# CommonRoad/commonroad-reactive-planner

Measured on AMD Instinct MI355X. Metric: candidate trajectories/sec (sample+cost+collision) per replan, higher is better.
Workload: dtype f64; 1 GPU; cfg3: DEU_Test-1_1_T-1, 31x31x63 grid, N=60, 51 obstacles (49 synthetic, seed 0); mode=draw, horizon_steps=60, n_obstacles=51, parallelism=one GPU, exchange=none

## Files before the change

### commonroad-reactive-planner_amd/csrc/rp_host.hip

```cpp
#include <hip/hip_runtime.h>
#include <hip/hip_ext.h>
#include <sched.h>

#include <algorithm>
#include <atomic>
#include <chrono>
#include <cmath>
#include <cstdio>
#include <cstdlib>
#include <cstring>
#include <mutex>
#include <new>
#include <string>
#include <unordered_map>
#include <vector>

#include "rp_kernels.h"
#include "rp_frontend.h"
#include "rp_corridor.h"
#include "rp_pool.h"

namespace {

constexpr int kBlocksPerCU = 4;
constexpr int kFoldPartials = 256;
constexpr int kFoldThreshold = 8192;
constexpr size_t kAutoMaterializeBytes = 64u << 20;
constexpr size_t kLdsTableLimit = 65536;
constexpr int kChunkMinWavesPerCU = 7;
constexpr int kCostMinPerCU = 832;
constexpr int kSweepMinPerCU = 512;
constexpr int kLazyCap[RP_LAZY_LEVELS] = {1024, 4096, 16384};
constexpr int kLazyOff[RP_LAZY_LEVELS] = {0, 1024, 5120};
constexpr int kLazyListWords = 21504;
constexpr uint32_t kLazyTarget[RP_LAZY_LEVELS] = {128, 1024, 8192};

using ResultBlock = FinalizeOut;

struct Options {
    int lanes = 0;
    int eval_block = 0;
    int cost_kernel = -1;
    int chunk_kernel = -1;
    int lazy = -1;
    int sweep = -1;
    int fused_lon = 1;
    int fused_lon_blocks = -1;
    int auto_materialize = 1;
    int stage_out = 1, row_padding = 1, row_align = 0, tail_split = 1;
    int table_window = 1;
    int fold_threshold = kFoldThreshold;
    int lon_publish = 1, inline_grids = 1, event_bracket = 0, winner_lanes_as_batch = 0, zero_copy = 1, coeff_groups = 1;
    int winner_skip_query = 1;
    int lazy_trace = 0, print_stamps = 0, timing = 0;
    int wait_mode = RP_WAIT_SPIN;
};
struct OptionDesc {
    const char *key;
    int Options::*field;
    const char *env;
    bool env_negates;
    int lo, hi;
};
const OptionDesc kOptionTable[] = {
    {"lanes", &Options::lanes, "RP_AMD_G", false, 0, 64},
    {"eval_block", &Options::eval_block, "RP_AMD_EVAL_BLOCK", false, 0, 256},
    {"cost_kernel", &Options::cost_kernel, "RP_AMD_COST_KERNEL", false, -1, 1},
    {"chunk_kernel", &Options::chunk_kernel, "RP_AMD_CHUNK_KERNEL", false, -1, 1},
    {"lazy", &Options::lazy, "RP_AMD_LAZY", false, -1, 1},
    {"sweep", &Options::sweep, "RP_AMD_SWEEP", false, -1, 1},
    {"fused_lon", &Options::fused_lon, "RP_AMD_NO_FUSED_LON", true, 0, 1},
    {"fused_lon_blocks", &Options::fused_lon_blocks, "RP_AMD_FUSED_LON_BLOCKS", false, -1, 1 << 20},
    {"auto_materialize", &Options::auto_materialize, "RP_AMD_NO_AUTO_MATERIALIZE", true, 0, 1},
    {"stage_out", &Options::stage_out, "RP_AMD_NO_STAGE_OUT", true, 0, 1},
    {"row_padding", &Options::row_padding, "RP_AMD_NO_ROW_PADDING", true, 0, 1},
    {"row_align", &Options::row_align, "RP_AMD_ROW_ALIGN", false, 0, 16},
    {"tail_split", &Options::tail_split, "RP_AMD_NO_TAIL_SPLIT", true, 0, 1},
    {"table_window", &Options::table_window, "RP_AMD_NO_TABLE_WINDOW", true, 0, 1},
    {"fold_threshold", &Options::fold_threshold, "RP_AMD_FOLD_THRESHOLD", false, 1, 1 << 30},
    {"lon_publish", &Options::lon_publish, "RP_AMD_NO_LON_PUBLISH", true, 0, 1},
    {"inline_grids", &Options::inline_grids, "RP_AMD_NO_INLINE_GRIDS", true, 0, 1},
    {"event_bracket", &Options::event_bracket, "RP_AMD_EVENT_BRACKET", false, 0, 1},
    {"winner_lanes_as_batch", &Options::winner_lanes_as_batch, "RP_AMD_WINNER_G_AS_BATCH", false, 0, 1},
    {"winner_skip_query", &Options::winner_skip_query, "RP_AMD_NO_WINNER_SKIP_QUERY", true, 0, 1},
    {"zero_copy", &Options::zero_copy, "RP_AMD_NO_ZERO_COPY", true, 0, 1},
    {"coeff_groups", &Options::coeff_groups, "RP_AMD_NO_COEFF_GROUPS", true, 0, 1},
    {"lazy_trace", &Options::lazy_trace, "RP_AMD_LAZY_TRACE", false, 0, 1},
    {"print_stamps", &Options::print_stamps, "RP_AMD_PRINT_STAMPS", false, 0, 1},
    {"timing", &Options::timing, "RP_AMD_TIMING", false, 0, 1},
    {"wait_mode", &Options::wait_mode, "RP_AMD_WAIT_MODE", false, RP_WAIT_SPIN, RP_WAIT_EVENT},
};
const OptionDesc *find_option(const char *key) {
    if (!key) return nullptr;
    for (const OptionDesc &d : kOptionTable)
        if (std::strcmp(d.key, key) == 0) return &d;
    return nullptr;
}
void options_from_environment(Options &o) {
    for (const OptionDesc &d : kOptionTable) {
        const char *e = d.env ? std::getenv(d.env) : nullptr;
        if (!e) continue;
        const int v = d.env_negates ? 0 : std::atoi(e);
        if (v >= d.lo && v <= d.hi) o.*(d.field) = v;
    }
}

}

struct rp_ctx {
    Options opt;
    int device = 0;
    hipStream_t stream = nullptr;
    std::string err;
    int num_cus = 256;
    int profiling = 0;
    unsigned long long calls = 0;
    hipEvent_t ev0 = nullptr, ev1 = nullptr;
    bool time_next_launch = false, timed_by_launch = false;

// ... 50 lines not shown
    std::chrono::steady_clock::time_point plan_t0;
    bool epilogue_dirty = false;
    struct Pending {
        bool active = false, cin = false, skip_eval = false, ticket = false, done = false, time_valid = false, mat = false, coeffs = false;
        unsigned long long seq = 0;
        int grid = 0;
        KArgs ka{};
        std::chrono::steady_clock::time_point tp0, tp1;
    } pending;
    struct LevelState {
        Pending pending;
        std::vector<char> staged;
        bool staged_on_device = false, last_rows_on_device = false;
        int last_G = 0, last_block = 0, last_kernel = 0, last_lazy = 0;
        size_t last_fused_lds = 0;
        int grid_index = 0;
    };
    std::vector<LevelState> chain;
    int chain_total = 0;
    unsigned long long *d_gate = nullptr;
    unsigned long long *d_sweep = nullptr;
    struct ChainInputs {
        rp_params p; rp_cost cost; std::vector<rp_grids> grids; std::vector<std::vector<double>> T, L, D; std::vector<std::vector<int32_t>> tl;
        int want = 0;
    } chain_in;
    int last_level = 0;
    char *d_result = nullptr, *h_result = nullptr, *h_result_dev = nullptr;
    size_t cap_result = 0;
    int64_t *d_single = nullptr, *h_single = nullptr;
    unsigned long long *d_debug = nullptr;
    unsigned long long seq = 0;
    bool spin_wait = true;
    hipEvent_t ev_done = nullptr;
    long long wait_fallbacks = 0;

    bool have_last = false, last_mat = false, last_coeffs = false;
    std::unordered_map<const void *, hipFunction_t> functions;
    std::vector<double> fast_buf;
    bool timing = false;
    double t_sum[6] = {0, 0, 0, 0, 0, 0};
    unsigned long long t_calls = 0;
    bool t_warm = false;
    std::chrono::steady_clock::time_point t_entry;
    bool last_rows_on_device = false;
    int last_G = 0;
    int last_block = 0;
    size_t last_fused_lds = 0;
    KArgs last{};
    KArgsG kargs_g{};
    KArgsGL kargs_gl{};
    bool grids_pending = false;
    char *h_arena = nullptr, *h_arena_dev = nullptr;
    int64_t arena_cap = 0;
    const double *cin_lon = nullptr, *cin_lat = nullptr;
    int64_t cin_groups = 0;
    const int32_t *cin_group_of = nullptr;
    int64_t cin_count = -1;
};

namespace {

int fail(rp_ctx *c, int code, const std::string &msg) {
    if (c) c->err = msg;
    return code;
}

// ... 75 lines not shown
        if (f && hipExtModuleLaunchKernel(f, (uint32_t)grid * (uint32_t)block, 1, 1, (uint32_t)block, 1, 1, lds, c->stream, nullptr, extra,
                                          c->ev0, c->ev1, 0) == hipSuccess) {
            c->timed_by_launch = true;
            return;
        }
        (void)hipGetLastError();
    }
    if (!f || hipModuleLaunchKernel(f, (unsigned)grid, 1, 1, (unsigned)block, 1, 1, (unsigned)lds, c->stream, nullptr, extra) != hipSuccess) {
        (void)hipGetLastError();
        void *args[] = {const_cast<void *>(args_block)};
        (void)hipLaunchKernel(kernel, dim3(grid), dim3(block), args, lds, c->stream);
    }
}

int collision_level(const KArgs &ka) {
    if (!ka.has_obstacles || (ka.flags & RP_FLAG_SKIP_COLLISION)) return 0;
    return (ka.obs.n_sobb + ka.obs.n_tri + ka.obs.n_circ) > 0 ? 2 : 1;
}

const void *sweep_kernel_fn(bool cin, int coll, bool one_chunk) {
    if (cin) {
        if (coll == 2) return one_chunk ? (const void *)rp_eval_kernel<16, false, true, 2, true, false, false, RP_BLOCK, true> : (const void *)rp_eval_kernel<16, false, true, 2, false, false, false, RP_BLOCK, true>;
        return one_chunk ? (const void *)rp_eval_kernel<16, false, true, 1, true, false, false, RP_BLOCK, true> : (const void *)rp_eval_kernel<16, false, true, 1, false, false, false, RP_BLOCK, true>;
    }
    if (coll == 2) return one_chunk ? (const void *)rp_eval_kernel<16, false, false, 2, true, false, false, RP_BLOCK, true> : (const void *)rp_eval_kernel<16, false, false, 2, false, false, false, RP_BLOCK, true>;
    return one_chunk ? (const void *)rp_eval_kernel<16, false, false, 1, true, false, false, RP_BLOCK, true> : (const void *)rp_eval_kernel<16, false, false, 1, false, false, false, RP_BLOCK, true>;
}

const void *chunk_kernel_fn(bool low, int coll) {
    if (low) return coll == 2 ? (const void *)rp_chunk_kernel<true, 2> : (coll == 1 ? (const void *)rp_chunk_kernel<true, 1> : (const void *)rp_chunk_kernel<true, 0>);
    return coll == 2 ? (const void *)rp_chunk_kernel<false, 2> : (coll == 1 ? (const void *)rp_chunk_kernel<false, 1> : (const void *)rp_chunk_kernel<false, 0>);
}

template <int G, bool MAT, bool CIN, int COLL, bool STAGE>
void launch_eval_tcs(rp_ctx *c, const KArgs &ka, int grid, size_t lds, int block = RP_BLOCK) {
    if constexpr (G == 16 && !STAGE) {
        if (block == 64) {
            if (ka.N + 1 <= G) launch_kargs(c, (const void *)rp_eval_kernel<G, MAT, CIN, COLL, true, false, false, 64>, grid, 64, lds, ka);
            else launch_kargs(c, (const void *)rp_eval_kernel<G, MAT, CIN, COLL, false, false, false, 64>, grid, 64, lds, ka);
            return;
        }
    }
    if (ka.N + 1 <= G) launch_kargs(c, (const void *)rp_eval_kernel<G, MAT, CIN, COLL, true, STAGE, false>, grid, RP_BLOCK, lds, ka);
    else launch_kargs(c, (const void *)rp_eval_kernel<G, MAT, CIN, COLL, false, STAGE, false>, grid, RP_BLOCK, lds, ka);
}

constexpr int kFusedLonG = 16;
constexpr size_t kFusedLonLdsLimit = 61440;
int fused_lon_max_blocks(const rp_ctx *c) {
    if (c->opt.fused_lon_blocks >= 0) return c->opt.fused_lon_blocks;
    return c->num_cus * 4;
}

size_t fused_lon_lds(const rp_ctx *c, const KArgs &ka, int64_t count, int G, bool cin, bool mat, int *pairs) {
    if (count <= 0 || !(G == kFusedLonG || (G == 64 && mat && ka.N + 1 <= 64) || (G == 32 && mat && ka.N + 1 <= 32))) return 0;
    const int gpb = RP_BLOCK / G;
    if ((count + gpb - 1) / gpb > (int64_t)fused_lon_max_blocks(c)) return 0;
    const int P = cin ? gpb : std::min<int64_t>(gpb, ((int64_t)gpb + ka.nD - 2) / ka.nD + 1);
    const size_t slot_bytes = ka.has_obstacles ? (size_t)ka.obs.n_clus * ka.obs.clus_per * RP_SLOT_ROW * sizeof(double) : 0;
    const size_t bytes = (size_t)ka.table_words * sizeof(double) + slot_bytes +
                         (size_t)P * ((size_t)PF_STRIDE * (size_t)(ka.N + 1) * sizeof(double) + sizeof(PairHdr) + sizeof(int) + sizeof(double)) + 16;
    if (bytes > kFusedLonLdsLimit) return 0;
    *pairs = P;
    return (bytes + 15) & ~(size_t)15;
}

template <bool MAT, bool CIN, int COLL>
void launch_eval_fused_c(rp_ctx *c, const KArgs &ka, int grid, size_t lds, int lanes) {
// ... 850 lines not shown
int rp_last_path(const rp_ctx *c) { return c ? c->last_lazy : 0; }
int rp_last_kernel(const rp_ctx *c) { return c ? c->last_kernel : 0; }

int rp_set_collision_path(rp_ctx *c, int mode) {
    if (!c) return RP_EINVAL;
    if (mode < RP_COLLISION_AUTO || mode > RP_COLLISION_TIMED) return fail(c, RP_EINVAL, "rp_set_collision_path: unknown mode");
    if (mode != c->collision_mode) { c->lazy_skip = c->lazy_penalty = 0; c->path_regime = -1; }
    c->collision_mode = mode;
    return RP_OK;
}

int rp_set_profiling(rp_ctx *c, int enable) {
    if (!c) return RP_EINVAL;
    c->profiling = enable < 0 ? 0 : enable;
    return RP_OK;
}

int rp_set_option(rp_ctx *c, const char *key, int64_t value) {
    if (!c) return RP_EINVAL;
    if (c->pending.active) return fail(c, RP_ESTATE, "rp_set_option: a plan is in flight on this context (rp_plan_wait first)");
    const OptionDesc *d = find_option(key);
    if (!d) return fail(c, RP_EINVAL, std::string("rp_set_option: unknown option '") + (key ? key : "(null)") + "'");
    if (value < d->lo || value > d->hi) return fail(c, RP_EINVAL, std::string("rp_set_option: value out of range for '") + key + "'");
    c->opt.*(d->field) = (int)value;
    c->timing = c->opt.timing != 0;
    c->spin_wait = c->opt.wait_mode != RP_WAIT_EVENT;
    c->lazy_skip = c->lazy_penalty = 0; c->path_regime = -1;
    return RP_OK;
}

int rp_get_option(const rp_ctx *c, const char *key, int64_t *value) {
    if (!c || !value) return RP_EINVAL;
    if (key && std::strcmp(key, "wait_fallbacks") == 0) { *value = c->wait_fallbacks; return RP_OK; }
    const OptionDesc *d = find_option(key);
    if (!d) return RP_EINVAL;
    *value = c->opt.*(d->field);
    return RP_OK;
}

int rp_set_wait_mode(rp_ctx *c, int mode) { return rp_set_option(c, "wait_mode", mode); }
int rp_get_wait_mode(const rp_ctx *c) { return c ? c->opt.wait_mode : RP_WAIT_SPIN; }

int rp_set_reference(rp_ctx *c, int32_t n, const double *ref_pos, const double *ref_theta, const double *ref_curv,
                     const double *ref_curv_d, const double *ref_x, const double *ref_y, double proj_domain_d_limit) {
    if (!c) return RP_EINVAL;
    if (c->pending.active) return fail(c, RP_ESTATE, "rp_set_reference: a plan is in flight on this context (rp_plan_wait first)");
    if (n < 2 || !ref_pos || !ref_theta || !ref_curv || !ref_curv_d || !ref_x || !ref_y)
        return fail(c, RP_EINVAL, "rp_set_reference: need n >= 2 and six non-null tables");
    for (int i = 0; i + 1 < n; ++i)
        if (!(ref_pos[i + 1] > ref_pos[i])) return fail(c, RP_EINVAL, "rp_set_reference: ref_pos must be strictly increasing");
    HIP_TRY(c, hipSetDevice(c->device));
    std::vector<double> t((size_t)TB_ROWS * (size_t)n);
    std::memcpy(&t[(size_t)TB_POS * n], ref_pos, sizeof(double) * n);
    std::memcpy(&t[(size_t)TB_THETA * n], ref_theta, sizeof(double) * n);
    std::memcpy(&t[(size_t)TB_CURV * n], ref_curv, sizeof(double) * n);
    std::memcpy(&t[(size_t)TB_CURV_D * n], ref_curv_d, sizeof(double) * n);
    std::memcpy(&t[(size_t)TB_X * n], ref_x, sizeof(double) * n);
    std::memcpy(&t[(size_t)TB_Y * n], ref_y, sizeof(double) * n);
    double *tx = &t[(size_t)TB_TX * n], *ty = &t[(size_t)TB_TY * n];
    std::vector<double> ux(n - 1), uy(n - 1);
    for (int i = 0; i + 1 < n; ++i) {
        double ex = ref_x[i + 1] - ref_x[i], ey = ref_y[i + 1] - ref_y[i];
        double ln = std::sqrt(ex * ex + ey * ey);
        if (!(ln > 0.0)) return fail(c, RP_EINVAL, "rp_set_reference: duplicate polyline vertices");
        ux[i] = ex / ln; uy[i] = ey / ln;
    }
// ... 1256 lines not shown
```

### commonroad-reactive-planner_amd/csrc/rp_kernels.h

```cpp
#pragma once

#include "rp_device.h"

#define RP_BLOCK 256
#ifndef RP_COPY_OUT_STORE
#define RP_COPY_OUT_STORE(p, v)                                                                                   \
    __builtin_nontemporal_store(*reinterpret_cast<const __attribute__((ext_vector_type(2))) double *>(&(v)),        \
                                reinterpret_cast<__attribute__((ext_vector_type(2))) double *>(p))
#endif
#ifndef RP_WRITE_THROUGH
#ifndef RP_BRANCHFREE_CONSTRAINTS
#define RP_BRANCHFREE_CONSTRAINTS 1
#endif
#define RP_WRITE_THROUGH 1
#endif
#ifndef RP_LATE_KERNARGS
#define RP_LATE_KERNARGS 1
#endif
#ifndef RP_WAVES_PER_SIMD
#define RP_WAVES_PER_SIMD 3
#endif

struct KArgs {
    double dt;
    int32_t N, factor, time_step0, low_vel_mode, lon_mode;
    uint32_t constraint_mask, flags;
    double x0_lon[3], x0_lat[3], x0_orientation;
    double wheelbase, wb_rear_axle, half_length, half_width, ego_radius;
    double a_max, v_switch, v_delta_max, kappa_max;
    double c_yaw;
    double c_kdot;
    int32_t cost_kind, has_speed, has_s, partials_cap;
    double w_a, desired_speed, desired_d, desired_s;
    int32_t nT, nL, nD, grids_inline;
    const double *T;
    const int32_t *traj_len;
    const double *L;
    const double *D;
    const double *lon_coeffs;
    const double *lat_coeffs;
    const int32_t *traj_len_c;
    const int32_t *pair_of;
    const int32_t *group_first;
    int64_t cand_begin, count;
    const int64_t *single_index;
    const int32_t *index_list;
    const uint32_t *list_count;
    int32_t list_cap;
    int32_t tail_split;
    struct LazyCtl *lazy_ctl;
    unsigned long long *sweep_init;
    unsigned long long *sweep_bound;
    int32_t partials_first, pad_sweep_;
// ... 1298 lines not shown
template <bool COEFFS_IN>
__device__ __forceinline__ void fetch_lateral(const KArgs &a, int64_t gidx, CandIn &ci, int64_t hdr_pair0) {
    int64_t pair;
    if (COEFFS_IN) {
        const double *pt = a.lat_coeffs + 6 * gidx;
#pragma unroll
        for (int k = 0; k < 6; ++k) ci.v[k] = pt[k];
        pair = pair_index<true>(a, gidx);
    } else {
        const uint32_t g32 = (uint32_t)gidx, nd = (uint32_t)a.nD;
        const uint32_t p32 = g32 / nd;
        pair = p32;
        ci.v[0] = grid_base(a)[a.nT + a.nL + (int)(g32 - p32 * nd)];
    }
    ci.pair_slot = pair - hdr_pair0;
}

__device__ __forceinline__ void fetch_header(const PairHdr *hdrs, CandIn &ci) {
    const PairHdr h = hdrs[ci.pair_slot];
    ci.lat_T = h.lat_T;
    ci.s0 = h.s0;
    ci.pre_reason = h.pre_reason;
    ci.L = h.L;
}

template <bool COEFFS_IN>
__device__ __forceinline__ CandIn fetch_candidate(const KArgs &a, int64_t gidx, const PairHdr *hdrs, int64_t hdr_pair0) {
    CandIn ci;
    fetch_lateral<COEFFS_IN>(a, gidx, ci, hdr_pair0);
    fetch_header(hdrs, ci);
    return ci;
}

template <int G, bool MAT, bool COEFFS_IN, int COLL, bool ONE_CHUNK, bool STAGE_OUT, bool LON_FUSED, int BLOCK = RP_BLOCK, bool SWEEP = false>
__global__ __launch_bounds__(BLOCK, RP_WAVES_PER_SIMD) void rp_eval_kernel(const KArgsG ag) {
    static_assert(!SWEEP || (G == 16 && !MAT && COLL != 0 && !STAGE_OUT && !LON_FUSED && BLOCK == RP_BLOCK), "the sweep's variant");
    const KArgs &a = ag.k;
    extern __shared__ double lds_out[];
    static_assert(!(LON_FUSED && STAGE_OUT), "the single-launch variant stores state rows directly");
    constexpr bool RP_WT = LON_FUSED && RP_WRITE_THROUGH;
    constexpr bool RP_NT = MAT && !LON_FUSED && !STAGE_OUT;
    touch_kernargs<10>();

    const int tid = threadIdx.x;
    RP_STAMP(0);
    RP_TL(0);
    const int lane = tid & 63;
    const int gl = lane & (G - 1);
    const int gbase = lane & ~(G - 1);
    static_assert(BLOCK == RP_BLOCK || (!LON_FUSED && !STAGE_OUT), "smaller workgroups: plain two-kernel variants only");
    constexpr int GPB = BLOCK / G;
    constexpr int GPW = 64 / G;
    constexpr int PFN = COLL ? PF_FIELDS : PF_COS_REF;
    const int wave_in_block = tid >> 6;
    const int group_in_wave = gbase / G;
    const int grp = tid / G;

    if (level_gate_closed(a.gate, a.gate_seq, a.gate_level)) return;
    if (a.single_index && *a.single_index < 0) {
        if (a.host_seq && a.ticket_if_none && tid == 0) __hip_atomic_store(a.host_seq, a.seq_value, __ATOMIC_RELEASE, __HIP_MEMORY_SCOPE_SYSTEM);
        return;
    }
    const int64_t wave_first = ((int64_t)blockIdx.x * GPB) + (int64_t)wave_in_block * GPW;
    int64_t count_ = a.single_index ? 1 : a.count;
    if (!LON_FUSED && a.index_list) {
        const uint32_t lc = *a.list_count;
        count_ = (int64_t)(lc < (uint32_t)a.list_cap ? lc : (uint32_t)a.list_cap);
        if ((int64_t)blockIdx.x * GPB >= count_) {
            if (a.partials) {
// ... 14 lines not shown
    if (sweep) {
        const int64_t sl = wave_first + group_in_wave;
        const bool v0 = sl < count;
        const int64_t slc = v0 ? sl : 0;
        const uint32_t st0 = a.status[slc];
        const double cs0 = a.cost[slc];
        const unsigned long long bound = __hip_atomic_load(a.sweep_bound, __ATOMIC_RELAXED, __HIP_MEMORY_SCOPE_AGENT);
        sweep_need = v0 && RP_STATUS_LABEL(st0) == RP_LABEL_FEASIBLE && cs0 == cs0 && cost_key(cs0) <= bound;
        __shared__ int sh_sweep_any;
        if (tid == 0) sh_sweep_any = 0;
        __syncthreads();
        if (__ballot(sweep_need) != 0 && lane == 0) sh_sweep_any = 1;
        __syncthreads();
        if (!sh_sweep_any) {
            if (a.partials) {
                const Partials bp = partials_at(a.partials, a.partials_cap, a.partials_first + (int)blockIdx.x);
                if (tid == 0) { bp.cost[0] = 0.0; bp.idx[0] = -1; }
                if (tid >= 8 && tid < 8 + RP_PARTIAL_CNT) bp.cnt[tid - 8] = 0u;
            }
            return;
        }
    }

    __shared__ GroupScratch sh_grp[GPB];
    __shared__ double sh_best_cost[GPB];
    __shared__ long long sh_best_idx[GPB];
    __shared__ int sh_cnt[10];

    const double *prof_base = a.profile;
    const PairHdr *hdr_base = a.pair_hdr;
    int64_t pair0 = a.pair_begin;
    CandIn cin;
    ProfStep pf0;
    const double *slot_lds = nullptr;
    if (LON_FUSED) {
        const int n0 = a.N + 1;
        double *const lds_tab = lds_out;
        double *const lds_prof = lds_tab + a.table_words;
        PairHdr *const lds_hdr = reinterpret_cast<PairHdr *>(lds_prof + (size_t)a.lds_pairs * PF_STRIDE * (size_t)n0);
        int *const lds_flags = reinterpret_cast<int *>(lds_hdr + a.lds_pairs);
        double *const lds_T = reinterpret_cast<double *>(lds_flags + ((a.lds_pairs + 1) & ~1));
        double *const lds_slot = reinterpret_cast<double *>((reinterpret_cast<uintptr_t>(lds_T + a.lds_pairs) + 15) & ~(uintptr_t)15);
        const int n_slots = (COLL == 2 && a.has_obstacles) ? a.obs.n_clus * a.obs.clus_per : 0;
        slot_lds = lds_slot;
        const int64_t s_first = (int64_t)blockIdx.x * GPB;
        const int64_t s_last = (s_first + GPB <= count ? s_first + GPB : count) - 1;
        const int64_t g_first = a.single_index ? *a.single_index : a.cand_begin + (s_first < count ? s_first : 0);
        const int64_t g_last = a.single_index ? g_first : a.cand_begin + (s_last >= s_first ? s_last : s_first);
        const int64_t p_first = COEFFS_IN ? g_first : (int64_t)((uint32_t)g_first / (uint32_t)a.nD);
        const int64_t p_last = COEFFS_IN ? g_last : (int64_t)((uint32_t)g_last / (uint32_t)a.nD);
        int P = (int)(p_last - p_first) + 1;
        P = P > a.lds_pairs ? a.lds_pairs : P;
        const int items = P * n0;
        __shared__ double sh_gT[GPB], sh_gL[GPB], sh_gD[GPB];
        __shared__ int sh_gtl[GPB];
        const int64_t slot0 = wave_first + group_in_wave;
        const int64_t g0 = a.single_index ? g_first : a.cand_begin + (slot0 < count ? slot0 : (wave_first < count ? wave_first : s_first));
        int j = lane;
        LonPairIn lin;
        double g_T = 0.0, g_L = 0.0, g_D = 0.0;
        int g_tl = 0;
        if (COEFFS_IN) {
            fetch_lateral<COEFFS_IN>(a, g0, cin, p_first);
            if (j < items) lin = lon_pair_fetch<COEFFS_IN>(a, p_first + (int)((uint32_t)j / (uint32_t)n0));
        } else {
            cin.pair_slot = (int64_t)((uint32_t)g0 / (uint32_t)a.nD) - p_first;
// ... 165 lines not shown
                RP_STAMP(22);
                const bool bounded = item_bound(it, bx, by, bR);
                RP_STAMP(23);
                if (!bounded) {
                    if (sub == 0 && dyn_here) atomicOr(mask_word(it, PF_NEAR), ~0ull);
                    continue;
                }
                if (dyn_here) {
                    uint64_t m = 0;
                    if (first) {
                        const double dx = f_cx - bx, dy = f_cy - by, rr = bR + f_r;
                        if (dx * dx + dy * dy <= rr * rr * 1.000001) m |= 1ull << (sub < 63 ? sub : 63);
                    }
                    for (int jo = sub + lanes_per_item; jo < ob.n_dyn; jo += lanes_per_item) {
                        const gcdouble o = dyn + (size_t)jo * ob.n_steps + kk;
                        const double dx = o[0] - bx, dy = o[plane] - by, rr = bR + o[6 * plane];
                        if (dx * dx + dy * dy <= rr * rr * 1.000001) m |= 1ull << (jo < 63 ? jo : 63);
                    }
                    if (m) atomicOr(mask_word(it, PF_NEAR), m);
                }
            }
            __syncthreads();
        }
        RP_STAMP(10);
        prof_base = lds_prof;
        hdr_base = lds_hdr;
        pair0 = p_first;
        pf0 = load_profile_item<PFN>(lds_prof + ((size_t)cin.pair_slot * (size_t)n0 + (size_t)(gl <= a.N ? gl : a.N)) * PF_STRIDE);
    } else {
        const int64_t slot0 = wave_first + group_in_wave;
        const int64_t ls0 = slot0 < count ? slot0 : (wave_first < count ? wave_first : (a.index_list ? (int64_t)blockIdx.x * GPB : 0));
        const int64_t g0 = a.single_index ? *a.single_index : (a.index_list ? (int64_t)a.index_list[ls0] : a.cand_begin + ls0);
        cin = fetch_candidate<COEFFS_IN>(a, g0, hdr_base, pair0);
        const int32_t ps0 = (int32_t)(pair_index<COEFFS_IN>(a, g0) - pair0);
        const int32_t pw0 = __builtin_amdgcn_readfirstlane(ps0);
        const uint32_t n80 = (uint32_t)(a.N + 1) * 8u;
        pf0 = load_profile<PFN, G == 16>(reinterpret_cast<const char *>(prof_base + ((size_t)pw0 * PF_FIELDS) * (size_t)(a.N + 1)),
                           (uint32_t)(ps0 - pw0) * PF_FIELDS * n80 + (uint32_t)(gl <= a.N ? gl : a.N) * 8u, n80);
    }

    if (!LON_FUSED) {
        if (tid < 10) sh_cnt[tid] = 0;
        if (tid < GPB) { sh_best_cost[tid] = 0.0; sh_best_idx[tid] = -1; }
        __syncthreads();
    }
    RP_STAMP(1);

    typedef const KArgs __attribute__((address_space(4))) *kargs_cptr;
    kargs_cptr ap_late = (LON_FUSED || MAT) ? (kargs_cptr)__builtin_amdgcn_kernarg_segment_ptr() : (kargs_cptr)&a;
    if (RP_LATE_KERNARGS && LON_FUSED) asm volatile("" : "+s"(ap_late));
    const KArgs __attribute__((address_space(4))) &al = *ap_late;
    const int N = al.N, n = N + 1;
    const int nchunks = ONE_CHUNK ? 1 : (n + G - 1) / G;
    const double dt = al.dt;
    const bool draw = (al.flags & RP_FLAG_DRAW_ALL) != 0;
    const bool low = al.low_vel_mode != 0;
    const uint32_t cm = al.constraint_mask;
    const int mid = n / 2;
    double *const gs_poly = sh_grp[grp].poly;
    double *const gs_last = sh_grp[grp].last;

    auto cost_terms = [&](int i, double acc, double v, double s, double d, double th_cl) -> double {
        double e, cst;
        e = al.w_a * acc; cst = e * e;
        e = 0.25 * (al.desired_d - d); cst = __builtin_fma(e, e, cst);
        e = 0.25 * fabs(th_cl); cst = __builtin_fma(e, e, cst);
        if (al.has_speed) { e = 5.0 * (v - al.desired_speed); cst = __builtin_fma(e, e, cst); }
        if (al.has_s) { e = 0.25 * (al.desired_s - s); cst = __builtin_fma(e, e, cst); }
        if (i == N) {
            e = 20.0 * (al.desired_d - d); cst = __builtin_fma(e, e, cst);
            e = 5.0 * fabs(th_cl); cst = __builtin_fma(e, e, cst);
            if (al.has_speed) { e = v - al.desired_speed; cst += 50.0 * (e * e); }
            if (al.has_s) { e = 20.0 * (al.desired_s - s); cst = __builtin_fma(e, e, cst); }
        }
        if (i == mid && al.has_speed) { e = v - al.desired_speed; cst += 100.0 * (e * e); }
        return cst;
    };

    if (wave_first < count) {
        const int64_t w0 = wave_first;
        const int64_t slot = w0 + group_in_wave;
        const bool valid = slot < count && sweep_need;
        const int64_t gidx = al.single_index ? *al.single_index
                             : ((!LON_FUSED && al.index_list) ? (int64_t)al.index_list[valid ? slot : w0] : al.cand_begin + (valid ? slot : w0));

        const int L = cin.L;
        const double s0 = cin.s0;
        const uint32_t pre_reason = (uint32_t)cin.pre_reason;
        const int32_t pair_slot_ = (int32_t)(pair_index<COEFFS_IN>(al, gidx) - pair0);
        const int32_t pair_w = __builtin_amdgcn_readfirstlane(pair_slot_);
        const uint32_t n8p = (uint32_t)n * 8u;
        const char *const pbase = reinterpret_cast<const char *>(prof_base + ((size_t)pair_w * PF_FIELDS) * (size_t)n);
        const uint32_t poff8 = (uint32_t)(pair_slot_ - pair_w) * PF_FIELDS * n8p;
        ProfStep pf = pf0;
        if (!LON_FUSED) {
            Poly lat;
            if (COEFFS_IN) lat = {cin.v[0], cin.v[1], cin.v[2], cin.v[3], cin.v[4], cin.v[5]};
            else lat = quintic_coeffs(al.x0_lat[0], al.x0_lat[1], al.x0_lat[2], cin.v[0], 0.0, 0.0, cin.lat_T);
            if (gl == 0) park_poly(gs_poly, lat);
        }
        RP_STAMP(2);

        int fail_step = -1, ood_step = -1;
        uint32_t fail_reason = RP_REASON_NONE;
        bool collide = false;
        double cost_acc = 0.0;

        bool alive = valid && pre_reason == RP_REASON_NONE;
        if (__ballot(alive) != 0) {
            double theta_carry = al.x0_orientation;
            double kappa_carry = 0.0;
            double cumx = 0.0, cumy = 0.0;
            const bool store_ok = MAT && valid && pre_reason == RP_REASON_NONE;
            const int ns = (MAT && !STAGE_OUT) ? al.row_stride : n;
            constexpr bool SPLIT_OK = MAT && !STAGE_OUT && !LON_FUSED && G == 16;
            const int tail_m = SPLIT_OK ? al.tail_split : 0;
            const uint32_t cand8 = (uint32_t)state_block_doubles(ns, tail_m) * 8u;
            char *const obase = !MAT ? nullptr
                                : (STAGE_OUT ? reinterpret_cast<char *>(lds_out + (size_t)(wave_in_block * GPW) * RP_N_ARRAYS * (size_t)n)
                                             : reinterpret_cast<char *>(al.states) + (size_t)w0 * (size_t)cand8);
            const uint32_t n8 = (uint32_t)ns * 8u;
            const uint32_t lane_off8 = (uint32_t)group_in_wave * (STAGE_OUT ? RP_N_ARRAYS * n8 : cand8);
            constexpr bool ROW_MULV = LON_FUSED;
            constexpr bool LATE_STORE = MAT && !STAGE_OUT;
            uint32_t n8v = n8;
            auto row_at = [&](uint32_t off8, int row) -> double * {
                return reinterpret_cast<double *>(obase + (size_t)(ROW_MULV ? __umul24((uint32_t)row, n8v) + off8 : off8 + (uint32_t)row * n8));
            };

#pragma nounroll
            for (int c = 0; c < nchunks; ++c) {
                const int base = c * G;
                const int i = base + gl;
                const bool live = i <= N;
                const bool act = i < L;
                if (ROW_MULV) asm volatile("" : "+v"(n8v));

                if (!ONE_CHUNK && c > 0) {
                    if (LON_FUSED) pf = load_profile_item<PFN>(prof_base + ((size_t)pair_slot_ * (size_t)n + (size_t)(live ? i : N)) * PF_STRIDE);
                    else pf = load_profile<PFN, G == 16>(pbase, poff8 + (uint32_t)(live ? i : N) * 8u, n8p);
                }
                double s = pf.f[PF_S], sd = pf.f[PF_SD], sdd = pf.f[PF_SDD];
                const double inv_sd = pf.f[PF_INV_SD], th_ref = pf.f[PF_TH_REF];
                const double k_r = pf.f[PF_KR], k_r_d = pf.f[PF_KRD];
                const double px = pf.f[PF_PX], py = pf.f[PF_PY], nx = pf.f[PF_NX], ny = pf.f[PF_NY];
                const bool s_in_dom = pf.f[PF_INDOM] != 0.0;

                constexpr bool SKIP_EXTENDED = !(MAT && COLL == 0);
                double d = 0.0, dd = 0.0, ddd = 0.0, th_cl = 0.0, th_gl = 0.0, cos_gl = 1.0, sin_gl = 0.0;
                double kappa = 0.0, v = 0.0, acc = 0.0, kdot = 0.0, x = 0.0, y = 0.0;
                uint64_t near_sta_cell = 0;
                if (!SKIP_EXTENDED || __any(act)) {
                    const double t = (double)i * dt;
                    const double tau = low ? s - s0 : t;
                    d = poly_pos(gs_poly, tau); dd = poly_vel(gs_poly, tau); ddd = poly_acc(gs_poly, tau);
                    if (fabs(dd) < RP_EPS) dd = 0.0;
                    if (!LATE_STORE && store_ok && act) {
                        const uint32_t off8 = lane_off8 + (uint32_t)i * 8u;
                        st_row<RP_WT, RP_NT>(row_at(off8, RP_S), s);
                        st_row<RP_WT, RP_NT>(row_at(off8, RP_S_DOT), sd);
                        st_row<RP_WT, RP_NT>(row_at(off8, RP_S_DDOT), sdd);
                        st_row<RP_WT, RP_NT>(row_at(off8, RP_D), d);
                        st_row<RP_WT, RP_NT>(row_at(off8, RP_D_DOT), dd);
                        st_row<RP_WT, RP_NT>(row_at(off8, RP_D_DDOT), ddd);
                    }
                    RP_STAMP(3);

                    const bool moving = inv_sd > 0.0;
                    double dp, dpp;
                    if (!low) {
                        dp = dd * inv_sd;
                        const double ddot = ddd - dp * sdd;
                        dpp = ddot * inv_sd * inv_sd;
                    } else {
                        dp = dd;
                        dpp = ddd;
                    }

                    const bool use_atan = moving || low;
                    th_cl = rp_atan(dp);
                    th_gl = th_cl + th_ref;
                    const double w2 = __builtin_fma(dp, dp, 1.0);
                    double cosT = rp_rsqrt(w2);
                    double secT = w2 * cosT;
                    double tanT = dp;
                    if (__any(act && !use_atan)) {
                        const uint64_t mv = group_ballot<G>(use_atan && act, gbase);
                        const uint64_t below = mv & ((1ull << gl) - 1ull);
                        const int src = below ? 63 - __clzll(below) : 0;
                        const double th_from = group_bcast<G>(th_gl, src);
                        if (!use_atan) {
                            th_gl = below ? th_from : theta_carry;
                            th_cl = th_gl - th_ref;
                        }
                        double sn, cs;
                        rp_sincos(th_cl, &sn, &cs);
                        const double sc = rp_rcp(cs);
                        cosT = use_atan ? cosT : cs;
                        secT = use_atan ? secT : sc;
                        tanT = use_atan ? tanT : sn * sc;
                    }
                    const double sinT = tanT * cosT;
                    cos_gl = heading_cos(pf.f[PF_COS_REF], pf.f[PF_SIN_REF], cosT, sinT);
                    sin_gl = heading_sin(pf.f[PF_COS_REF], pf.f[PF_SIN_REF], cosT, sinT);
                    RP_STAMP(5);

                    const double oneKrD = 1.0 - k_r * d;
                    const double q = cosT * rp_rcp(oneKrD);
                    const double kterm = frenet_kterm(k_r_d, d, k_r, dp);
                    kappa = frenet_kappa(dpp, kterm, tanT, cosT, q, k_r);
                    const double f = oneKrD * secT;
                    v = sd * f;
                    acc = frenet_acc(sdd, f, sd, secT, oneKrD, tanT, kappa, k_r, kterm);

                    double th_prev = lane_prev(th_gl), ka_prev = lane_prev(kappa);
                    if (gl == 0) { th_prev = theta_carry; ka_prev = kappa_carry; }
                    const double dth = i > 0 ? th_gl - th_prev : 0.0;
                    kdot = i > 0 ? kappa - ka_prev : 0.0;
                    RP_STAMP(6);

    #if RP_BRANCHFREE_CONSTRAINTS
                    uint32_t reason = RP_REASON_NONE;
                    {
                        const double a_max = al.a_max, v_switch = al.v_switch, kappa_max = al.kappa_max;
                        const double wk = al.wheelbase * kappa;
                        const bool bad_yaw = fabs(rint(dth * al.c_yaw)) > kappa_max * v * 1e5;
                        const bool bad_kd = fabs(kdot) > al.c_kdot * __builtin_fma(wk, wk, 1.0);
                        const bool fast = v > v_switch;
                        const double acc_l = fast ? acc * v : acc, acc_r = fast ? a_max * v_switch : a_max;
                        const bool bad_acc = !((-a_max <= acc) & (acc_l <= acc_r));
                        const bool bad_v = v < -RP_EPS, bad_k = fabs(kappa) > kappa_max;
                        reason = (((cm & RP_CHECK_ACCELERATION) != 0) & bad_acc) ? RP_REASON_ACCELERATION : reason;
                        reason = (((cm & RP_CHECK_KAPPA_DOT) != 0) & bad_kd) ? RP_REASON_KAPPA_DOT : reason;
                        reason = (((cm & RP_CHECK_YAW_RATE) != 0) & bad_yaw) ? RP_REASON_YAW_RATE : reason;
                        reason = (((cm & RP_CHECK_KAPPA) != 0) & bad_k) ? RP_REASON_KAPPA : reason;
                        reason = (((cm & RP_CHECK_VELOCITY) != 0) & bad_v) ? RP_REASON_VELOCITY : reason;
                        reason = act ? reason : RP_REASON_NONE;
                    }
    #else
                    uint32_t reason = RP_REASON_NONE;
                    if (act) {
                        const double wk = al.wheelbase * kappa;
                        const bool bad_yaw = fabs(rint(dth * al.c_yaw)) > al.kappa_max * v * 1e5;
                        const bool bad_kd = fabs(kdot) > al.c_kdot * __builtin_fma(wk, wk, 1.0);
                        const bool ok_acc = (-al.a_max <= acc) && (v > al.v_switch ? acc * v <= al.a_max * al.v_switch : acc <= al.a_max);
                        if ((cm & RP_CHECK_VELOCITY) && v < -RP_EPS) reason = RP_REASON_VELOCITY;
                        else if ((cm & RP_CHECK_KAPPA) && fabs(kappa) > al.kappa_max) reason = RP_REASON_KAPPA;
                        else if ((cm & RP_CHECK_YAW_RATE) && bad_yaw) reason = RP_REASON_YAW_RATE;
                        else if ((cm & RP_CHECK_KAPPA_DOT) && bad_kd) reason = RP_REASON_KAPPA_DOT;
                        else if ((cm & RP_CHECK_ACCELERATION) && !ok_acc) reason = RP_REASON_ACCELERATION;
                    }
    #endif
                    if (__any(reason != RP_REASON_NONE)) {
                        const uint64_t fm = group_ballot<G>(reason != RP_REASON_NONE, gbase);
                        const int fl = fm ? __ffsll((unsigned long long)fm) - 1 : 0;
                        const uint32_t r_first = (uint32_t)__shfl((int)reason, fl, G);
                        if (fm && fail_step < 0) { fail_step = base + fl; fail_reason = r_first; }
                        if (!draw && fail_step >= 0) alive = false;
                        if (__ballot(alive) == 0) break;
                    }
                    RP_STAMP(7);

                    const bool in_dom = s_in_dom && fabs(d) <= al.proj_d_limit;
                    x = px + d * nx; y = py + d * ny;
                    if (__any(act && !in_dom) || ood_step >= 0) {
                        const uint64_t om = group_ballot<G>(act && !in_dom, gbase);
                        if (om && ood_step < 0) ood_step = base + __ffsll((unsigned long long)om) - 1;
                        if (ood_step >= 0 && i >= ood_step) { x = 0.0; y = 0.0; }
                    }
                    if (act) {
                        if (!LATE_STORE && store_ok) {
                            const uint32_t off8 = lane_off8 + (uint32_t)i * 8u;
                            st_row<RP_WT, RP_NT>(row_at(off8, RP_X), x);
                            st_row<RP_WT, RP_NT>(row_at(off8, RP_Y), y);
                            st_row<RP_WT, RP_NT>(row_at(off8, RP_THETA), th_gl);
                            st_row<RP_WT, RP_NT>(row_at(off8, RP_V), v);
                            st_row<RP_WT, RP_NT>(row_at(off8, RP_A), acc);
                            st_row<RP_WT, RP_NT>(row_at(off8, RP_KAPPA), kappa);
                            st_row<RP_WT, RP_NT>(row_at(off8, RP_KAPPA_DOT), kdot);
                            st_row<RP_WT, RP_NT>(row_at(off8, RP_THETA_CL), th_cl);
                        }
                        cost_acc += cost_terms(i, acc, v, s, d, th_cl);
                    }
                    if (COLL == 2 && live && alive && fail_step < 0 && ood_step < 0 && !collide && act)
                        near_sta_cell = static_grid_mask(al.obs.grid, al.obs.gx0, al.obs.gy0, al.obs.ginv, al.obs.gnx, al.obs.gny,
                                                         x + al.wb_rear_axle * cos_gl, y + al.wb_rear_axle * sin_gl);
                }
                const bool cell_wanted = COLL == 2 && live && alive && fail_step < 0 && ood_step < 0 && !collide;
                RP_STAMP(8);

                const int ll = L - 1 - base;
                const bool take = (ll >= 0 && ll < G);
                if (__any(take && L < n)) {
                    if (!COLL) rp_sincos(th_gl, &sin_gl, &cos_gl);
                    if (take && gl == ll) {
                        double *o = gs_last;
                        o[0] = x; o[1] = y; o[2] = th_gl; o[3] = v; o[4] = acc; o[5] = kappa; o[6] = kdot;
// ... 71 lines not shown
                        char *const tbase = obase + (size_t)(lane_off8 + (uint32_t)(RP_N_ARRAYS * tail_m) * 8u + (uint32_t)gl * 8u);
                        const bool lo = gl < 8;
                        auto pair_store = [&](int q, double r0, double r1) {
                            const double up = dpp_f64<DPP_ROW_SHR8, 0xf>(r1);
                            st_row<RP_WT, RP_NT>(reinterpret_cast<double *>(tbase + q * 128), lo ? r0 : up);
                        };
                        pair_store(0, x, y); pair_store(1, th_gl, v); pair_store(2, acc, kappa); pair_store(3, kdot, s);
                        pair_store(4, d, th_cl); pair_store(5, sd, sdd); pair_store(6, dd, ddd);
                    }
                } else
                if (LATE_STORE && store_ok && i < ns) {
                    const uint32_t off8 = lane_off8 + (uint32_t)i * 8u;
                    st_row<RP_WT, RP_NT>(row_at(off8, RP_X), x);
                    st_row<RP_WT, RP_NT>(row_at(off8, RP_Y), y);
                    st_row<RP_WT, RP_NT>(row_at(off8, RP_THETA), th_gl);
                    st_row<RP_WT, RP_NT>(row_at(off8, RP_V), v);
                    st_row<RP_WT, RP_NT>(row_at(off8, RP_A), acc);
                    st_row<RP_WT, RP_NT>(row_at(off8, RP_KAPPA), kappa);
                    st_row<RP_WT, RP_NT>(row_at(off8, RP_KAPPA_DOT), kdot);
                    st_row<RP_WT, RP_NT>(row_at(off8, RP_S), s);
                    st_row<RP_WT, RP_NT>(row_at(off8, RP_D), d);
                    st_row<RP_WT, RP_NT>(row_at(off8, RP_THETA_CL), th_cl);
                    st_row<RP_WT, RP_NT>(row_at(off8, RP_S_DOT), sd);
                    st_row<RP_WT, RP_NT>(row_at(off8, RP_S_DDOT), sdd);
                    st_row<RP_WT, RP_NT>(row_at(off8, RP_D_DOT), dd);
                    st_row<RP_WT, RP_NT>(row_at(off8, RP_D_DDOT), ddd);
                }
                RP_STAMP(9);

                if (COLL) {
                    const bool want = live && alive && fail_step < 0 && ood_step < 0 && !collide;
                    bool hit = false;
                    constexpr bool masked = !COEFFS_IN;
                    const uint64_t near_dyn = double_as_mask(pf.f[PF_NEAR]);
                    const double ego_cx = x + al.wb_rear_axle * cos_gl, ego_cy = y + al.wb_rear_axle * sin_gl;
                    const uint64_t near_sta = want ? near_sta_cell : 0;
                    const bool ask = want && ((!masked && al.obs.n_dyn > 0) || (near_dyn | near_sta) != 0);
                    RP_STAMP(44);
#ifdef RP_WALK_COUNT
                    if (a.debug && !a.single_index && blockIdx.x == RP_STAMP_BLOCK && threadIdx.x == RP_STAMP_THREAD) rp_walk_dbg = a.debug + 40;
#endif
                    if (__any(ask)) {
                        ObsTables ob;
                        ob.sobb = al.obs.sobb; ob.tri = al.obs.tri; ob.circ = al.obs.circ; ob.dyn = al.obs.dyn;
                        ob.clus = al.obs.clus; ob.clus_info = al.obs.clus_info;
                        ob.n_sobb = al.obs.n_sobb; ob.n_tri = al.obs.n_tri; ob.n_circ = al.obs.n_circ; ob.n_dyn = al.obs.n_dyn;
                        ob.n_steps = al.obs.n_steps; ob.dyn_t0 = al.obs.dyn_t0; ob.n_clus = al.obs.n_clus; ob.clus_per = al.obs.clus_per;
                        ob.dyn_rmax_all = al.obs.dyn_rmax_all;
                        const Obb ego = {ego_cx, ego_cy, cos_gl, sin_gl, al.half_length, al.half_width};
                        RP_STAMP(45);
                        hit = pose_collides<masked, COLL == 2, LON_FUSED && COLL == 2, true, !MAT>(ob, ego, al.ego_radius, al.time_step0 + i * al.factor, ask,
                                                                                             near_dyn, near_sta, slot_lds) && ask;
                    }
                    RP_STAMP(46);
                    collide |= group_ballot<G>(hit, gbase) != 0;
                }
                RP_STAMP(11);
            }
        }
        RP_STAMP(12);
        if (MAT && STAGE_OUT) {
            const uint64_t okmask = __ballot(valid && pre_reason == RP_REASON_NONE);
            if (okmask) {
                const int blk2 = (RP_N_ARRAYS * n) >> 1;
                const double2 *src = reinterpret_cast<const double2 *>(lds_out + (size_t)(wave_in_block * GPW) * RP_N_ARRAYS * (size_t)n);
                double2 *dst = reinterpret_cast<double2 *>(al.states + ((size_t)w0 * RP_N_ARRAYS) * (size_t)n);
                for (int k = lane; k < GPW * blk2; k += 64) {
// ... 842 lines not shown
```

Measured before the change: 455.5 million candidates/s.

## Stage per-pair reference profile rows in LDS for the two-kernel eval path

Adds a PROF_LDS kernel variant that cooperatively copies each workgroup's longitudinal profile rows from global memory into LDS once, in batched loads, transposed to a strided per-step layout. The per-step loop then reads profile fields from LDS as needed, instead of reloading them from global memory for every chunk. This is meant to cut repeated global profile traffic and register pressure in the materialized, non-coefficient path. In exchange it adds LDS allocation (capped at 32KB), which may lower occupancy, plus a prologue copy. An option can disable it.

Result: faster. 464.3 million candidates/s (median of 6 runs) (+1.9%).

```diff
diff --git a/commonroad-reactive-planner_amd/csrc/rp_host.hip b/commonroad-reactive-planner_amd/csrc/rp_host.hip
--- a/commonroad-reactive-planner_amd/csrc/rp_host.hip
+++ b/commonroad-reactive-planner_amd/csrc/rp_host.hip
@@ -52,6 +52,7 @@
     int fold_threshold = kFoldThreshold;
     int lon_publish = 1, inline_grids = 1, event_bracket = 0, winner_lanes_as_batch = 0, zero_copy = 1, coeff_groups = 1;
     int winner_skip_query = 1;
+    int profile_lds = 1;
     int lazy_trace = 0, print_stamps = 0, timing = 0;
     int wait_mode = RP_WAIT_SPIN;
 };
@@ -85,6 +86,7 @@
     {"winner_skip_query", &Options::winner_skip_query, "RP_AMD_NO_WINNER_SKIP_QUERY", true, 0, 1},
     {"zero_copy", &Options::zero_copy, "RP_AMD_NO_ZERO_COPY", true, 0, 1},
     {"coeff_groups", &Options::coeff_groups, "RP_AMD_NO_COEFF_GROUPS", true, 0, 1},
+    {"profile_lds", &Options::profile_lds, "RP_AMD_NO_PROFILE_LDS", true, 0, 1},
     {"lazy_trace", &Options::lazy_trace, "RP_AMD_LAZY_TRACE", false, 0, 1},
     {"print_stamps", &Options::print_stamps, "RP_AMD_PRINT_STAMPS", false, 0, 1},
     {"timing", &Options::timing, "RP_AMD_TIMING", false, 0, 1},
@@ -201,6 +203,7 @@
     unsigned long long seq = 0;
     bool spin_wait = true;
     hipEvent_t ev_done = nullptr;
+    long long prof_lds_launches = 0;
     long long wait_fallbacks = 0;
 
     bool have_last = false, last_mat = false, last_coeffs = false;
@@ -342,8 +345,30 @@
     return coll == 2 ? (const void *)rp_chunk_kernel<false, 2> : (coll == 1 ? (const void *)rp_chunk_kernel<false, 1> : (const void *)rp_chunk_kernel<false, 0>);
 }
 
+constexpr size_t kProfLdsLimit = 32768;
+size_t prof_lds_bytes(const rp_ctx *c, const KArgs &ka, int G, int block, int *pairs) {
+    if (!c->opt.profile_lds || G != 16 || block != RP_BLOCK || ka.N + 1 <= G || ka.single_index || ka.index_list || ka.nD <= 0) return 0;
+    const int gpb = RP_BLOCK / G;
+    const int P = (int)std::min<int64_t>(gpb, ((int64_t)gpb + ka.nD - 2) / ka.nD + 1);
+    const size_t bytes = (size_t)P * PF_STRIDE * (size_t)(ka.N + 1) * sizeof(double);
+    if (bytes > kProfLdsLimit) return 0;
+    *pairs = P;
+    return bytes;
+}
+
 template <int G, bool MAT, bool CIN, int COLL, bool STAGE>
 void launch_eval_tcs(rp_ctx *c, const KArgs &ka, int grid, size_t lds, int block = RP_BLOCK) {
+    if constexpr (G == 16 && MAT && !CIN && !STAGE) {
+        int pairs = 0;
+        const size_t bytes = prof_lds_bytes(c, ka, G, block, &pairs);
+        if (bytes) {
+            KArgs kp = ka;
+            kp.lds_pairs = pairs;
+            launch_kargs(c, (const void *)rp_eval_kernel<G, MAT, CIN, COLL, false, false, false, RP_BLOCK, false, true>, grid, RP_BLOCK, bytes, kp);
+            ++c->prof_lds_launches;
+            return;
+        }
+    }
     if constexpr (G == 16 && !STAGE) {
         if (block == 64) {
             if (ka.N + 1 <= G) launch_kargs(c, (const void *)rp_eval_kernel<G, MAT, CIN, COLL, true, false, false, 64>, grid, 64, lds, ka);
@@ -1260,6 +1285,7 @@
 int rp_get_option(const rp_ctx *c, const char *key, int64_t *value) {
     if (!c || !value) return RP_EINVAL;
     if (key && std::strcmp(key, "wait_fallbacks") == 0) { *value = c->wait_fallbacks; return RP_OK; }
+    if (key && std::strcmp(key, "profile_lds_launches") == 0) { *value = c->prof_lds_launches; return RP_OK; }
     const OptionDesc *d = find_option(key);
     if (!d) return RP_EINVAL;
     *value = c->opt.*(d->field);
diff --git a/commonroad-reactive-planner_amd/csrc/rp_kernels.h b/commonroad-reactive-planner_amd/csrc/rp_kernels.h
--- a/commonroad-reactive-planner_amd/csrc/rp_kernels.h
+++ b/commonroad-reactive-planner_amd/csrc/rp_kernels.h
@@ -19,6 +19,9 @@
 #endif
 #ifndef RP_WAVES_PER_SIMD
 #define RP_WAVES_PER_SIMD 3
+#endif
+#ifndef RP_PROF_LDS_WAVES
+#define RP_PROF_LDS_WAVES 3
 #endif
 
 struct KArgs {
@@ -1383,9 +1386,12 @@
     return ci;
 }
 
-template <int G, bool MAT, bool COEFFS_IN, int COLL, bool ONE_CHUNK, bool STAGE_OUT, bool LON_FUSED, int BLOCK = RP_BLOCK, bool SWEEP = false>
-__global__ __launch_bounds__(BLOCK, RP_WAVES_PER_SIMD) void rp_eval_kernel(const KArgsG ag) {
+template <int G, bool MAT, bool COEFFS_IN, int COLL, bool ONE_CHUNK, bool STAGE_OUT, bool LON_FUSED, int BLOCK = RP_BLOCK, bool SWEEP = false,
+          bool PROF_LDS = false>
+__global__ __launch_bounds__(BLOCK, PROF_LDS ? RP_PROF_LDS_WAVES : RP_WAVES_PER_SIMD) void rp_eval_kernel(const KArgsG ag) {
     static_assert(!SWEEP || (G == 16 && !MAT && COLL != 0 && !STAGE_OUT && !LON_FUSED && BLOCK == RP_BLOCK), "the sweep's variant");
+    static_assert(!PROF_LDS || (G == 16 && !COEFFS_IN && !ONE_CHUNK && !STAGE_OUT && !LON_FUSED && BLOCK == RP_BLOCK && !SWEEP),
+                  "profile rows in LDS: 16-lane grid plans of the two-kernel path, 256-thread workgroups");
     const KArgs &a = ag.k;
     extern __shared__ double lds_out[];
     static_assert(!(LON_FUSED && STAGE_OUT), "the single-launch variant stores state rows directly");
@@ -1466,6 +1472,7 @@
     int64_t pair0 = a.pair_begin;
     CandIn cin;
     ProfStep pf0;
+    int32_t plds0 = 0;
     const double *slot_lds = nullptr;
     if (LON_FUSED) {
         const int n0 = a.N + 1;
@@ -1697,11 +1704,37 @@
         const int64_t ls0 = slot0 < count ? slot0 : (wave_first < count ? wave_first : (a.index_list ? (int64_t)blockIdx.x * GPB : 0));
         const int64_t g0 = a.single_index ? *a.single_index : (a.index_list ? (int64_t)a.index_list[ls0] : a.cand_begin + ls0);
         cin = fetch_candidate<COEFFS_IN>(a, g0, hdr_base, pair0);
-        const int32_t ps0 = (int32_t)(pair_index<COEFFS_IN>(a, g0) - pair0);
-        const int32_t pw0 = __builtin_amdgcn_readfirstlane(ps0);
-        const uint32_t n80 = (uint32_t)(a.N + 1) * 8u;
-        pf0 = load_profile<PFN, G == 16>(reinterpret_cast<const char *>(prof_base + ((size_t)pw0 * PF_FIELDS) * (size_t)(a.N + 1)),
-                           (uint32_t)(ps0 - pw0) * PF_FIELDS * n80 + (uint32_t)(gl <= a.N ? gl : a.N) * 8u, n80);
+        if (PROF_LDS) {
+            const int n0 = a.N + 1;
+            const int64_t s_first = (int64_t)blockIdx.x * GPB, s_last = (s_first + GPB <= count ? s_first + GPB : count) - 1;
+            const uint32_t nd = (uint32_t)a.nD, p_first = (uint32_t)(a.cand_begin + s_first) / nd;
+            const int P = (int)((uint32_t)(a.cand_begin + s_last) / nd - p_first) + 1;
+            plds0 = (int32_t)((int64_t)p_first - pair0);
+            const int rows = (P < a.lds_pairs ? P : a.lds_pairs) * PFN;
+            const double *const src = prof_base + (size_t)plds0 * PF_FIELDS * (size_t)n0;
+            constexpr int WPB = BLOCK / 64, BATCH = 8;
+            for (int r0 = wave_in_block; r0 < rows; r0 += BATCH * WPB) {
+                for (int i = lane; i < n0; i += 64) {
+                    double v[BATCH];
+#pragma unroll
+                    for (int u = 0; u < BATCH; ++u) {
+                        const int r = r0 + u * WPB < rows ? r0 + u * WPB : rows - 1;
+                        v[u] = src[(size_t)((r / PFN) * PF_FIELDS + r % PFN) * (size_t)n0 + i];
+                    }
+#pragma unroll
+                    for (int u = 0; u < BATCH; ++u) {
+                        const int r = r0 + u * WPB;
+                        if (r < rows) lds_out[((r / PFN) * n0 + i) * PF_STRIDE + r % PFN] = v[u];
+                    }
+                }
+            }
+        } else {
+            const int32_t ps0 = (int32_t)(pair_index<COEFFS_IN>(a, g0) - pair0);
+            const int32_t pw0 = __builtin_amdgcn_readfirstlane(ps0);
+            const uint32_t n80 = (uint32_t)(a.N + 1) * 8u;
+            pf0 = load_profile<PFN, G == 16>(reinterpret_cast<const char *>(prof_base + ((size_t)pw0 * PF_FIELDS) * (size_t)(a.N + 1)),
+                               (uint32_t)(ps0 - pw0) * PF_FIELDS * n80 + (uint32_t)(gl <= a.N ? gl : a.N) * 8u, n80);
+        }
     }
 
     if (!LON_FUSED) {
@@ -1758,6 +1791,8 @@
         const char *const pbase = reinterpret_cast<const char *>(prof_base + ((size_t)pair_w * PF_FIELDS) * (size_t)n);
         const uint32_t poff8 = (uint32_t)(pair_slot_ - pair_w) * PF_FIELDS * n8p;
         ProfStep pf = pf0;
+        typedef const double __attribute__((address_space(3))) *lds_cdouble;
+        const uint32_t prow8 = PROF_LDS ? (uint32_t)(pair_slot_ - plds0) * (uint32_t)n * (uint32_t)(PF_STRIDE * 8) : 0u;
         if (!LON_FUSED) {
             Poly lat;
             if (COEFFS_IN) lat = {cin.v[0], cin.v[1], cin.v[2], cin.v[3], cin.v[4], cin.v[5]};
@@ -1801,15 +1836,15 @@
                 const bool act = i < L;
                 if (ROW_MULV) asm volatile("" : "+v"(n8v));
 
-                if (!ONE_CHUNK && c > 0) {
+                const lds_cdouble pit = (lds_cdouble)(const double *)(reinterpret_cast<const char *>(lds_out) + prow8 +
+                                                                      (uint32_t)(live ? i : N) * (uint32_t)(PF_STRIDE * 8));
+                auto prof = [&](int k) -> double { return PROF_LDS ? (k < PFN ? pit[k] : 0.0) : pf.f[k]; };
+                if (!PROF_LDS && !ONE_CHUNK && c > 0) {
                     if (LON_FUSED) pf = load_profile_item<PFN>(prof_base + ((size_t)pair_slot_ * (size_t)n + (size_t)(live ? i : N)) * PF_STRIDE);
                     else pf = load_profile<PFN, G == 16>(pbase, poff8 + (uint32_t)(live ? i : N) * 8u, n8p);
                 }
-                double s = pf.f[PF_S], sd = pf.f[PF_SD], sdd = pf.f[PF_SDD];
-                const double inv_sd = pf.f[PF_INV_SD], th_ref = pf.f[PF_TH_REF];
-                const double k_r = pf.f[PF_KR], k_r_d = pf.f[PF_KRD];
-                const double px = pf.f[PF_PX], py = pf.f[PF_PY], nx = pf.f[PF_NX], ny = pf.f[PF_NY];
-                const bool s_in_dom = pf.f[PF_INDOM] != 0.0;
+                double s = prof(PF_S), sd = prof(PF_SD), sdd = prof(PF_SDD);
+                const double inv_sd = prof(PF_INV_SD);
 
                 constexpr bool SKIP_EXTENDED = !(MAT && COLL == 0);
                 double d = 0.0, dd = 0.0, ddd = 0.0, th_cl = 0.0, th_gl = 0.0, cos_gl = 1.0, sin_gl = 0.0;
@@ -1843,6 +1878,7 @@
                     }
 
                     const bool use_atan = moving || low;
+                    const double th_ref = prof(PF_TH_REF);
                     th_cl = rp_atan(dp);
                     th_gl = th_cl + th_ref;
                     const double w2 = __builtin_fma(dp, dp, 1.0);
@@ -1866,10 +1902,12 @@
                         tanT = use_atan ? tanT : sn * sc;
                     }
                     const double sinT = tanT * cosT;
-                    cos_gl = heading_cos(pf.f[PF_COS_REF], pf.f[PF_SIN_REF], cosT, sinT);
-                    sin_gl = heading_sin(pf.f[PF_COS_REF], pf.f[PF_SIN_REF], cosT, sinT);
+                    const double cos_ref = prof(PF_COS_REF), sin_ref = prof(PF_SIN_REF);
+                    cos_gl = heading_cos(cos_ref, sin_ref, cosT, sinT);
+                    sin_gl = heading_sin(cos_ref, sin_ref, cosT, sinT);
                     RP_STAMP(5);
 
+                    const double k_r = prof(PF_KR), k_r_d = prof(PF_KRD);
                     const double oneKrD = 1.0 - k_r * d;
                     const double q = cosT * rp_rcp(oneKrD);
                     const double kterm = frenet_kterm(k_r_d, d, k_r, dp);
@@ -1926,8 +1964,8 @@
                     }
                     RP_STAMP(7);
 
-                    const bool in_dom = s_in_dom && fabs(d) <= al.proj_d_limit;
-                    x = px + d * nx; y = py + d * ny;
+                    const bool in_dom = prof(PF_INDOM) != 0.0 && fabs(d) <= al.proj_d_limit;
+                    x = prof(PF_PX) + d * prof(PF_NX); y = prof(PF_PY) + d * prof(PF_NY);
                     if (__any(act && !in_dom) || ood_step >= 0) {
                         const uint64_t om = group_ballot<G>(act && !in_dom, gbase);
                         if (om && ood_step < 0) ood_step = base + __ffsll((unsigned long long)om) - 1;
@@ -2065,7 +2103,7 @@
                     const bool want = live && alive && fail_step < 0 && ood_step < 0 && !collide;
                     bool hit = false;
                     constexpr bool masked = !COEFFS_IN;
-                    const uint64_t near_dyn = double_as_mask(pf.f[PF_NEAR]);
+                    const uint64_t near_dyn = double_as_mask(prof(PF_NEAR));
                     const double ego_cx = x + al.wb_rear_axle * cos_gl, ego_cy = y + al.wb_rear_axle * sin_gl;
                     const uint64_t near_sta = want ? near_sta_cell : 0;
                     const bool ask = want && ((!masked && al.obs.n_dyn > 0) || (near_dyn | near_sta) != 0);
```
